# vrgamegirl19/comfyui-vrgamedevgirl

Measured on AMD Instinct MI355X. Metric: Mpixels/s (grain+LUT+colormatch+sharpen) at 4K, higher is better.
Workload: dtype f32

## Files before the change

### comfyui-vrgamedevgirl_amd/csrc/vrg_apply_body.hpp

```cpp
#pragma once
#include "vrg_chain_stages.hpp"
#include "vrg_lanes.hpp"

namespace vrg {

#define VRG_APPLY_ROWS 60
constexpr int APPLY_ROWS = VRG_APPLY_ROWS;
constexpr int APPLY_COLS = 62;
static_assert(APPLY_ROWS % 3 == 0, "APPLY_ROWS must be a multiple of 3");

__device__ __forceinline__ float am_prev(float v) { return tap_prev(v); }
__device__ __forceinline__ float am_next(float v) { return tap_next(v); }

struct AmRow { float l[3], c[3], r[3]; };

#define VRG_APPLY_EARLY_LOAD 1
template <int STAGES, class MATH, bool GENERAL = true>
__device__ __forceinline__ void apply_march_body(uint32_t vblock, uint32_t vgrid, const px3* __restrict__ in, px3* __restrict__ out, int32_t H, int32_t W,
                                                 int32_t strips_x, int32_t segs_y, uint32_t total_waves, const ChainK& D, const MATH& PT) {
    const uint32_t groups = (total_waves + 3u) / 4u;
    const uint32_t per_xcd = (groups + 7u) / 8u;
    const int lane = threadIdx.x & 63;
    const bool zero = D.zero_border != 0;
    const int64_t ppf = (int64_t)H * W;
    const float n0[3] = {0.0f, 0.0f, 0.0f};
    for (uint32_t slot = vblock >> 3; slot < per_xcd; slot += (vgrid >> 3)) {
    const uint32_t grp = (vblock & 7u) * per_xcd + slot;
    if (grp >= groups) break;
    const uint32_t wv = (uint32_t)__builtin_amdgcn_readfirstlane((int)(grp * 4u + (threadIdx.x >> 6)));
    if (wv >= total_waves) break;
    const uint32_t strip = wv % (uint32_t)strips_x;
    const uint32_t rest = wv / (uint32_t)strips_x;
    const uint32_t seg = rest % (uint32_t)segs_y;
    const int64_t f = rest / (uint32_t)segs_y;
    int32_t x0 = (int32_t)strip * APPLY_COLS, y0 = (int32_t)seg * APPLY_ROWS;
    if (W >= APPLY_COLS) x0 = x0 < W - APPLY_COLS ? x0 : W - APPLY_COLS;
    if (H >= APPLY_ROWS) y0 = y0 < H - APPLY_ROWS ? y0 : H - APPLY_ROWS;
    const int32_t rows = H >= APPLY_ROWS ? APPLY_ROWS : H;
    const int32_t x = x0 - 1 + lane;
    const bool x_in = x >= 0 && x < W;
    const int32_t xc = x < 0 ? 0 : (x > W - 1 ? W - 1 : x);
    const bool stores = lane >= 1 && lane <= APPLY_COLS && x_in;
    const px3* fin = in + f * ppf;
    px3* fout = out + f * ppf;
    __amdgpu_buffer_rsrc_t frame_rsrc, in_rsrc;
    if (!GENERAL) {
        const uint64_t fb = reinterpret_cast<uint64_t>(fout);
        const uint64_t fbu = ((uint64_t)(uint32_t)__builtin_amdgcn_readfirstlane((int)(fb >> 32)) << 32) | (uint32_t)__builtin_amdgcn_readfirstlane((int)(uint32_t)fb);
        frame_rsrc = __builtin_amdgcn_make_buffer_rsrc(reinterpret_cast<void*>(fbu), 0, (int)(ppf * 12), 0x00020000);
        const uint64_t ib = reinterpret_cast<uint64_t>(fin);
        const uint64_t ibu = ((uint64_t)(uint32_t)__builtin_amdgcn_readfirstlane((int)(ib >> 32)) << 32) | (uint32_t)__builtin_amdgcn_readfirstlane((int)(uint32_t)ib);
        in_rsrc = __builtin_amdgcn_make_buffer_rsrc(reinterpret_cast<void*>(ibu), 0, (int)(ppf * 12), 0x00020000);
    }
    const FrameCtx FC = frame_ctx<STAGES>(D, f);
    const uint32_t x_bytes = (uint32_t)xc * 12u;
    const uint32_t store_bytes = stores ? (uint32_t)x * 12u : 0x80000000u;

    auto load = [&](int32_t y) {
        const int32_t yc = y < 0 ? 0 : (y > H - 1 ? H - 1 : y);
        if (!GENERAL) {
            typedef unsigned u3 __attribute__((ext_vector_type(3)));
            const u3 v = __builtin_amdgcn_raw_buffer_load_b96(in_rsrc, (int)x_bytes, (int)((uint32_t)(yc * W) * 12u), 0);
            return px3{__uint_as_float(v.x), __uint_as_float(v.y), __uint_as_float(v.z)};
        }
        return fin[(int64_t)yc * W + xc];
    };
    auto process = [&](const px3& v, int32_t y) {
        AmRow r;
        const float xi[3] = {v.r, v.g, v.b};
        float o[3];
        chain_apply_stages<STAGES, !GENERAL>(D, FC, xi, n0, o, PT);
        r.c[0] = o[0]; r.c[1] = o[1]; r.c[2] = o[2];
        if (zero) {
            asm volatile("" ::: "memory");
            const bool inside = x_in && y >= 0 && y < H;
#pragma unroll
            for (int c = 0; c < 3; ++c) r.c[c] = inside ? r.c[c] : 0.0f;
        }
#pragma unroll
        for (int c = 0; c < 3; ++c) {
            r.l[c] = am_prev(r.c[c]);
            r.r[c] = am_next(r.c[c]);
        }
        return r;
    };
    auto emit = [&](int32_t y, const AmRow& a, const AmRow& b, const AmRow& c) {
        float res[3];
        if (STAGES & VRG_STAGE_COLORMATCH) {
            const float p[3][3][3] = {{{a.l[0], a.c[0], a.r[0]}, {b.l[0], b.c[0], b.r[0]}, {c.l[0], c.c[0], c.r[0]}},
                                      {{a.l[1], a.c[1], a.r[1]}, {b.l[1], b.c[1], b.r[1]}, {c.l[1], c.c[1], c.r[1]}},
                                      {{a.l[2], a.c[2], a.r[2]}, {b.l[2], b.c[2], b.r[2]}, {c.l[2], c.c[2], c.r[2]}}};
            stencil_value3_unit<!GENERAL>(D.stencil_op, p, D.strength, D.zero_border, res);
        } else {
#pragma unroll
            for (int ch = 0; ch < 3; ++ch) {
                const float p[3][3] = {{a.l[ch], a.c[ch], a.r[ch]}, {b.l[ch], b.c[ch], b.r[ch]}, {c.l[ch], c.c[ch], c.r[ch]}};
                res[ch] = stencil_value(D.stencil_op, p, D.strength, D.zero_border);
            }
        }
        if (GENERAL) {
            if (stores && y < y0 + rows) fout[(int64_t)y * W + x] = px3{res[0], res[1], res[2]};
        } else {
            typedef unsigned u3 __attribute__((ext_vector_type(3)));
            __builtin_amdgcn_raw_buffer_store_b96(u3{__float_as_uint(res[0]), __float_as_uint(res[1]), __float_as_uint(res[2])}, frame_rsrc, (int)store_bytes,
                                                  (int)((uint32_t)(y * W) * 12u), 0);
        }
    };

    AmRow r0 = process(load(y0 - 1), y0 - 1);
    AmRow r1 = process(load(y0), y0);
    AmRow r2;
    const int32_t y1 = y0 + rows;
    px3 q = load(y0 + 1);
    if (!GENERAL && VRG_APPLY_EARLY_LOAD) {
        for (int32_t y = y0; y < y1; y += 3) {
            const px3 a = load(y + 2);
            r2 = process(q, y + 1);
            emit(y, r0, r1, r2);
            const px3 b = load(y + 3);
            r0 = process(a, y + 2);
            emit(y + 1, r1, r2, r0);
            q = load(y + 4);
            r1 = process(b, y + 3);
            emit(y + 2, r2, r0, r1);
        }
    } else {
        for (int32_t y = y0; y < y1; y += 3) {
            r2 = process(q, y + 1);
            q = load(y + 2);
            emit(y, r0, r1, r2);
            r0 = process(q, y + 2);
            q = load(y + 3);
            emit(y + 1, r1, r2, r0);
            r1 = process(q, y + 3);
            q = load(y + 4);
            emit(y + 2, r2, r0, r1);
        }
    }
    }
}


}
```

### comfyui-vrgamedevgirl_amd/csrc/vrg_torch_stats.hip

```cpp
#include <atomic>
#include "vrg_tstats_body.hpp"
#include "vrg_tstats_config.hpp"

namespace vrg {

template <class OP, class LOAD>
static __device__ __forceinline__ typename OP::acc_t ts_thread_reduce(LOAD X, int64_t n, int shift, bool vectorize, int T, int t, int tx,
                                                                      bool tail_ok) {
    constexpr int VEC = OP::VEC;
    typename OP::acc_t acc[VEC];
#pragma unroll
    for (int i = 0; i < VEC; ++i) acc[i] = OP::ident();
    if (vectorize) {
        int64_t start = 0, end = n;
        if (shift > 0) {
            if (tx >= shift && tx < VEC && tail_ok) acc[0] = OP::template reduce<true>(acc[0], X((int64_t)(tx - shift)));
            start = VEC - shift;
            end = n + shift - VEC;
        }
        for (int64_t idx = t; idx * VEC + VEC - 1 < end; idx += T) {
            const int64_t p = start + idx * VEC;
            acc[0] = OP::template reduce<false>(acc[0], X(p));
#pragma unroll
            for (int i = 1; i < VEC; ++i) acc[i] = OP::template reduce<true>(acc[i], X(p + i));
        }
        const int64_t tail_start = end - end % VEC;
        if (tail_ok && tail_start + tx < end) acc[0] = OP::template reduce<true>(acc[0], X(start + tail_start + tx));
    } else {
        int64_t idx = t;
        while (idx + (int64_t)(VEC - 1) * T < n) {
#pragma unroll
            for (int i = 0; i < VEC; ++i) acc[i] = OP::template reduce<true>(acc[i], X(idx + (int64_t)i * T));
            idx += (int64_t)T * VEC;
        }
#pragma unroll
        for (int i = 0; i < VEC; ++i) {
            if (idx < n) acc[i] = OP::template reduce<true>(acc[i], X(idx));
            idx += T;
        }
    }
#pragma unroll
    for (int i = 1; i < VEC; ++i) acc[0] = OP::combine(acc[0], acc[i]);
    return acc[0];
}

template <class OP, int WHICH>
__global__ void __launch_bounds__(512) k_tstats_plane(const float* __restrict__ lab, int64_t n, int64_t plane0, int chunk_frames, TsCfg cfg,
                                                      float factor, float eps, float* __restrict__ out) {
    __shared__ typename OP::acc_t lds[512];
    const int64_t plane = plane0 + blockIdx.x;
    const int64_t f = plane / 3;
    const int c = (int)(plane % 3);
    const int64_t o_in_call = (f % chunk_frames) * 3 + c;
    const int shift = cfg.vectorize ? (int)((o_in_call * n) % OP::VEC) : 0;
    const int rows = cfg.split ? cfg.bh : 1;
    const int T = cfg.bw * rows;
    const int t = threadIdx.x;
    const bool live = t < T;
    const float* base = lab + (size_t)f * (size_t)n * 3 + c;
    auto X = [base](int64_t p) { return base[(size_t)p * 3]; };
    typename OP::acc_t v = OP::ident();
    if (live) v = ts_thread_reduce<OP>(X, n, shift, cfg.vectorize != 0, T, t, t % cfg.bw, cfg.split ? (t / cfg.bw == 0) : true);
    v = ts_block_reduce<OP>(v, cfg.bw, cfg.bh, cfg.split != 0, t, live, lds);
    if (t == 0) {
        if constexpr (WHICH == 0) out[(size_t)f * 6 + c * 2] = v * factor;
        else out[(size_t)f * 6 + c * 2 + 1] = welf_std(v) + eps;
    }
}

template <int DEPTH>
__global__ void __launch_bounds__(256) k_tstats_rows(const float* __restrict__ lab, int64_t n, int64_t frames, int bw, int bh, TsRows* __restrict__ rows) {
    __shared__ Welf lds_w[256];
    tstats_rows_body<DEPTH>(blockIdx.x, lab, n, frames, bw, bh, rows, lds_w);
}

__global__ void __launch_bounds__(64) k_tstats_rows_finish(const TsRows* __restrict__ rows, int64_t frames, int bh, float factor, float eps,
                                                          float* __restrict__ out) {
    const int64_t i = (int64_t)blockIdx.x * 64 + threadIdx.x;
    if (i >= frames * 6) return;
    const int64_t f = i / 6;
    const int c = (int)(i % 6) >> 1, which = (int)(i & 1);
    if (which == 0) {
        float v[8];
        for (int r = 0; r < bh; ++r) v[r] = rows[f].m[c][r];
        for (int off = bh / 2; off > 0; off >>= 1)
            for (int ty = 0; ty < off; ++ty) v[ty] = MeanOp::combine(v[ty], v[ty + off]);
        out[(size_t)f * 6 + c * 2] = v[0] * factor;
    } else {
        Welf v[8];
        for (int r = 0; r < bh; ++r) v[r] = rows[f].w[c][r];
        for (int off = bh / 2; off > 0; off >>= 1)
            for (int ty = 0; ty < off; ++ty) v[ty] = WelfOp::combine(v[ty], v[ty + off]);
        out[(size_t)f * 6 + c * 2 + 1] = welf_std(v[0]) + eps;
    }
}

struct TsLaneRec { float mean, m2; int cnt; int pad; };
struct TsLanes { TsLaneRec w[3][2][512]; float m[3][512]; };
constexpr int TS_LANES_MAX_STEPS = 16384;

#define VRG_TS_LANES_DEPTH 8
#define VRG_TS_LANES_MEAN_DEPTH 12
#define VRG_TS_LANES_MAX_FRAMES 2

template <bool FUSED, bool FAST, int DEPTH>
static __device__ __forceinline__ bool ts_lane_chain(const float* __restrict__ ub, uint32_t lane_bytes, int steps, bool extra, const float2* __restrict__ tab,
                                                     Welf& acc, int& cnt) {
    bool bad = false;
    acc = WelfOp::ident();
    float xb[DEPTH];
    const int last = steps > 0 ? steps - 1 : 0;
    auto load = [&](int k) {
        const int kk = k < last ? k : last;
        return *reinterpret_cast<const float*>(reinterpret_cast<const char*>(ub + (size_t)kk * 3072) + lane_bytes);
    };
#pragma unroll
    for (int i = 0; i < DEPTH; ++i) xb[i] = load(i);
    int k0 = 0;
    for (; k0 + DEPTH <= steps; k0 += DEPTH) {
#pragma unroll
        for (int i = 0; i < DEPTH; ++i) {
            const float2 t = tab[k0 + i];
            ts_welf_update<FUSED, FAST>(acc, xb[i], t.x, t.y, bad);
            xb[i] = load(k0 + i + DEPTH);
        }
    }
#pragma unroll
    for (int i = 0; i < DEPTH; ++i)
        if (k0 + i < steps) {
            const float2 t = tab[k0 + i];
            ts_welf_update<FUSED, FAST>(acc, xb[i], t.x, t.y, bad);
        }
    cnt = steps;
    if (extra) {
        const float2 t = tab[steps];
        const float x = *reinterpret_cast<const float*>(reinterpret_cast<const char*>(ub + (size_t)steps * 3072) + lane_bytes);
        ts_welf_update<FUSED, FAST>(acc, x, t.x, t.y, bad);
        cnt = steps + 1;
    }
    return bad;
}

template <int DEPTH>
__global__ void __launch_bounds__(448) k_tstats_lanes(const float* __restrict__ lab, int64_t n, int64_t frames, TsLanes* __restrict__ recs) {
    extern __shared__ __attribute__((aligned(16))) float2 ts_rn_tab[];
    const int64_t w = blockIdx.x;
    const int64_t f = (w & 7) + 8 * (w >> 6);
    const int j = (int)((w >> 3) & 7);
    if (f >= frames) return;
    const int wave = __builtin_amdgcn_readfirstlane((int)(threadIdx.x >> 6)), lane = threadIdx.x & 63;
    const int t = 64 * j + lane;
    const int64_t nvw = n / 2, nvm = n / 4;
    const int64_t wsteps = nvw / 512;
    const bool wextra = (int64_t)t < nvw - wsteps * 512;
    for (int64_t i = threadIdx.x; i <= wsteps; i += 448) {
        const float nf = (float)(i + 1);
        ts_rn_tab[i] = float2{nf, 1.0f / nf};
    }
    __syncthreads();
    const float* base = lab + (size_t)f * (size_t)n * 3;
    TsLanes* R = recs + f;
    bool bad = false;
    Welf acc = WelfOp::ident();
    int cnt = 0;
    const bool fast = VRG_TS_MARKSTEIN && wsteps + 2 <= TS_MARKSTEIN_MAX_COUNT;
    const int c = wave >> 1, a = wave & 1;
    const float* ub = base + (wave < 6 ? a * 3 + c : 0);
    const uint32_t lane_bytes = (uint32_t)t * 24u;
    const int ws = (int)wsteps;
    if (wave < 6) {
        if (fast) bad = a ? ts_lane_chain<true, true, DEPTH>(ub, lane_bytes, ws, wextra, ts_rn_tab, acc, cnt) : ts_lane_chain<false, true, DEPTH>(ub, lane_bytes, ws, wextra, ts_rn_tab, acc, cnt);
        else if (a) ts_lane_chain<true, false, DEPTH>(ub, lane_bytes, ws, wextra, ts_rn_tab, acc, cnt);
        else ts_lane_chain<false, false, DEPTH>(ub, lane_bytes, ws, wextra, ts_rn_tab, acc, cnt);
    } else {
        float ma[3][4];
#pragma unroll
        for (int cc = 0; cc < 3; ++cc)
#pragma unroll
            for (int i = 0; i < 4; ++i) ma[cc][i] = 0.0f;
        auto mean_vec = [&](const f32x4& a0, const f32x4& a1, const f32x4& a2) {
            const float e[12] = {a0.x, a0.y, a0.z, a0.w, a1.x, a1.y, a1.z, a1.w, a2.x, a2.y, a2.z, a2.w};
#pragma unroll
            for (int i = 0; i < 4; ++i)
#pragma unroll
                for (int cc = 0; cc < 3; ++cc) ma[cc][i] = ma[cc][i] + e[i * 3 + cc];
        };
        constexpr int MD = VRG_TS_LANES_MEAN_DEPTH;
        const int64_t msteps = nvm / 512;
        const bool mextra = (int64_t)t < nvm - msteps * 512;
        const int64_t last = msteps > 0 ? msteps - 1 : 0;
        f32x4 mb[MD][3];
        auto mload = [&](int i, int64_t r) {
            const f32x4* q = reinterpret_cast<const f32x4*>(base + (size_t)(r * 512 + t) * 12);
            mb[i][0] = q[0]; mb[i][1] = q[1]; mb[i][2] = q[2];
        };
#pragma unroll
        for (int i = 0; i < MD; ++i) mload(i, i < last ? i : last);
        int64_t r0 = 0;
        for (; r0 + MD <= msteps; r0 += MD) {
#pragma unroll
            for (int i = 0; i < MD; ++i) {
                mean_vec(mb[i][0], mb[i][1], mb[i][2]);
                const int64_t nx = r0 + i + MD;
                mload(i, nx < last ? nx : last);
            }
        }
#pragma unroll
        for (int i = 0; i < MD; ++i)
            if (r0 + i < msteps) mean_vec(mb[i][0], mb[i][1], mb[i][2]);
        if (mextra) {
            const f32x4* q = reinterpret_cast<const f32x4*>(base + (size_t)(msteps * 512 + t) * 12);
            mean_vec(q[0], q[1], q[2]);
        }
#pragma unroll
        for (int cc = 0; cc < 3; ++cc) {
            float m = ma[cc][0];
            m = m + ma[cc][1];
            m = m + ma[cc][2];
            m = m + ma[cc][3];
            R->m[cc][t] = m;
        }
    }
    if (fast && __syncthreads_or(bad ? 1 : 0)) {
        if (wave < 6) {
            if (a) ts_lane_chain<true, false, DEPTH>(ub, lane_bytes, ws, wextra, ts_rn_tab, acc, cnt);
            else ts_lane_chain<false, false, DEPTH>(ub, lane_bytes, ws, wextra, ts_rn_tab, acc, cnt);
        }
    }
    if (wave < 6) R->w[c][a][t] = TsLaneRec{acc.mean, acc.m2, cnt, 0};
}

__global__ void __launch_bounds__(512) k_tstats_lanes_finish(const TsLanes* __restrict__ recs, int bw, int bh, float factor, float eps, float* __restrict__ out) {
    __shared__ Welf lds_w[512];
    float* lds_m = reinterpret_cast<float*>(lds_w);
    const int64_t f = blockIdx.x;
    const int t = threadIdx.x;
    const TsLanes* R = recs + f;
    float* o6 = out + (size_t)f * 6;
#pragma unroll
    for (int c = 0; c < 3; ++c) {
        float m = R->m[c][t];
        m = ts_block_reduce<MeanOp>(m, bw, bh, true, t, true, lds_m);
        if (t == 0) o6[c * 2] = m * factor;
    }
#pragma unroll
    for (int c = 0; c < 3; ++c) {
        const TsLaneRec r0 = R->w[c][0][t], r1 = R->w[c][1][t];
        const Welf w0{r0.mean, r0.m2, r0.cnt, (float)r0.cnt}, w1{r1.mean, r1.m2, r1.cnt, (float)r1.cnt};
        Welf w = WelfOp::combine(w0, w1);
        w = ts_block_reduce<WelfOp>(w, bw, bh, true, t, true, lds_w);
        if (t == 0) o6[c * 2 + 1] = welf_std(w) + eps;
    }
}

template <bool SPLIT, int DEPTH>
__global__ void __launch_bounds__(512) k_tstats_frame(const float* __restrict__ lab, int64_t n, int64_t frames, int bw, int bh, float factor,
                                                      float eps, float* __restrict__ out) {
    __shared__ Welf lds_w[512];
    if constexpr (!SPLIT) {
        const int64_t f = blockIdx.x;
        ts_frame_part<-1, DEPTH>(lab + (size_t)f * (size_t)n * 3, n, bw, bh, factor, eps, out + (size_t)f * 6, lds_w);
    } else {
        const int64_t w = blockIdx.x;
        const int64_t f = (w & 7) + 8 * (w >> 5);
        const int part = (int)((w >> 3) & 3);
        if (f >= frames) return;
        const float* base = lab + (size_t)f * (size_t)n * 3;
        float* o6 = out + (size_t)f * 6;
        switch (part) {
            case 0: ts_frame_part<0, DEPTH>(base, n, bw, bh, factor, eps, o6, lds_w); break;
            case 1: ts_frame_part<1, DEPTH>(base, n, bw, bh, factor, eps, o6, lds_w); break;
            case 2: ts_frame_part<2, DEPTH>(base, n, bw, bh, factor, eps, o6, lds_w); break;
            default: ts_frame_part<3, DEPTH>(base, n, bw, bh, factor, eps, o6, lds_w); break;
        }
    }
}

static int ts_launch_planes(const float* lab_call, int64_t n, int64_t o0, int64_t o1, int chunk_frames, float factor, float eps, float* out_call,
                            int num_mp, hipStream_t st) {
    const int64_t O = o1 - o0;
    if (O * n > ((int64_t)1 << 29) && O > 1) {
        const int64_t half = O / 2;
        int rc = ts_launch_planes(lab_call, n, o0, o0 + half, chunk_frames, factor, eps, out_call, num_mp, st);
        if (rc != VRG_OK) return rc;
        return ts_launch_planes(lab_call, n, o0 + half, o1, chunk_frames, factor, eps, out_call, num_mp, st);
    }
    if (O * n > ((int64_t)1 << 29)) return VRG_ERR_UNSUPPORTED;
    TsCfg cm, cw;
    if (!ts_config(O, n, 4, cm, num_mp) || !ts_config(O, n, 2, cw, num_mp)) return VRG_ERR_UNSUPPORTED;
    hipLaunchKernelGGL((k_tstats_plane<MeanOp, 0>), dim3((unsigned)O), dim3(512), 0, st, lab_call, n, o0, chunk_frames, cm, factor, eps, out_call);
    hipLaunchKernelGGL((k_tstats_plane<WelfOp, 1>), dim3((unsigned)O), dim3(512), 0, st, lab_call, n, o0, chunk_frames, cw, factor, eps, out_call);
    VRG_CHECK_LAUNCH();
    return VRG_OK;
}

#define VRG_TS_SPLIT_MAX_FRAMES 64
constexpr int64_t TS_SPLIT_MAX_FRAMES = VRG_TS_SPLIT_MAX_FRAMES;

#define VRG_TS_ROWS_DEPTH 4
#define VRG_TS_SPLIT_DEPTH 2
#define VRG_TS_WHOLE_DEPTH 1
#define VRG_TS_ROWS_MAX_FRAMES 32
constexpr int64_t TS_ROWS_MAX_FRAMES = VRG_TS_ROWS_MAX_FRAMES;

static int ts_launch_calls(const float* lab, int64_t n, int64_t count, int b, float eps, float* out, int num_mp, void* scratch, int64_t scratch_bytes,
                           hipStream_t st, bool prefer_lanes = false) {
    if (count <= 0 || b <= 0) return VRG_OK;
    const int64_t O = (int64_t)b * 3;
    const float factor = (float)O / (float)(O * n);
    if (O * n > ((int64_t)1 << 29)) {
        for (int64_t k = 0; k < count; ++k) {
            const int rc = ts_launch_planes(lab + (size_t)k * b * n * 3, n, 0, O, b, factor, eps, out + (size_t)k * b * 6, num_mp, st);
            if (rc != VRG_OK) return rc;
        }
        return VRG_OK;
    }
    TsCfg cm, cw;
    if (!ts_config(O, n, 4, cm, num_mp) || !ts_config(O, n, 2, cw, num_mp)) return VRG_ERR_UNSUPPORTED;
    const int64_t frames = count * b;
    const bool whole = (n % 4 == 0) && cm.vectorize && cw.vectorize && cm.split && cw.split && cm.bw * cm.bh == 512 && cw.bw * cw.bh == 512 &&
                       cm.bw == cw.bw;
    if (whole) {
#define VRG_TS_LANES 1
        if (VRG_TS_LANES && prefer_lanes && frames <= VRG_TS_LANES_MAX_FRAMES && scratch && scratch_bytes >= frames * (int64_t)sizeof(TsLanes) && cm.bh == cw.bh &&
            n / 1024 + 2 <= TS_LANES_MAX_STEPS && (reinterpret_cast<uintptr_t>(scratch) & 15) == 0) {
            TsLanes* recs = reinterpret_cast<TsLanes*>(scratch);
            const size_t lds = (size_t)(n / 1024 + 2) * sizeof(float2);
            static std::atomic<uint64_t> attr_devices{0};
            int device = 0;
            if (hipGetDevice(&device) != hipSuccess) return VRG_ERR_LAUNCH;
            const uint64_t bit = (device >= 0 && device < 64) ? (1ull << device) : 0;
            if (!(attr_devices.load(std::memory_order_acquire) & bit)) {
                if (hipFuncSetAttribute(reinterpret_cast<const void*>(k_tstats_lanes<VRG_TS_LANES_DEPTH>), hipFuncAttributeMaxDynamicSharedMemorySize,
                                        TS_LANES_MAX_STEPS * (int)sizeof(float2)) != hipSuccess)
                    return VRG_ERR_LAUNCH;
                attr_devices.fetch_or(bit, std::memory_order_release);
            }
            hipLaunchKernelGGL((k_tstats_lanes<VRG_TS_LANES_DEPTH>), dim3((unsigned)(64 * ((frames + 7) / 8))), dim3(448), lds, st, lab, n, frames, recs);
            hipLaunchKernelGGL(k_tstats_lanes_finish, dim3((unsigned)frames), dim3(512), 0, st, recs, cm.bw, cm.bh, factor, eps, out);
            VRG_CHECK_LAUNCH();
            return VRG_OK;
        }
        if (frames <= TS_ROWS_MAX_FRAMES && scratch && scratch_bytes >= frames * (int64_t)sizeof(TsRows) && cm.bh == cw.bh && cm.bh <= 8 && 256 % cm.bw == 0 &&
            (reinterpret_cast<uintptr_t>(scratch) & 15) == 0) {
            TsRows* rows = reinterpret_cast<TsRows*>(scratch);
            hipLaunchKernelGGL((k_tstats_rows<VRG_TS_ROWS_DEPTH>), dim3((unsigned)(64 * ((frames + 7) / 8))), dim3(256), 0, st, lab, n, frames, cm.bw, cm.bh, rows);
            hipLaunchKernelGGL(k_tstats_rows_finish, dim3((unsigned)((frames * 6 + 63) / 64)), dim3(64), 0, st, rows, frames, cm.bh, factor, eps, out);
            VRG_CHECK_LAUNCH();
            return VRG_OK;
        }
        const bool split = frames <= TS_SPLIT_MAX_FRAMES;
        if (split) {
            hipLaunchKernelGGL((k_tstats_frame<true, VRG_TS_SPLIT_DEPTH>), dim3((unsigned)(32 * ((frames + 7) / 8))), dim3(512), 0, st, lab, n, frames, cm.bw,
                               cm.bh, factor, eps, out);
        } else {
            const int64_t per = num_mp > 0 ? num_mp : 256;
            for (int64_t f0 = 0; f0 < frames; f0 += per) {
                const int64_t nf = frames - f0 < per ? frames - f0 : per;
                hipLaunchKernelGGL((k_tstats_frame<false, VRG_TS_WHOLE_DEPTH>), dim3((unsigned)nf), dim3(512), 0, st, lab + (size_t)f0 * (size_t)n * 3, n, nf,
                                   cm.bw, cm.bh, factor, eps, out + (size_t)f0 * 6);
            }
        }
    } else {
        hipLaunchKernelGGL((k_tstats_plane<MeanOp, 0>), dim3((unsigned)(frames * 3)), dim3(512), 0, st, lab, n, (int64_t)0, b, cm, factor, eps, out);
        hipLaunchKernelGGL((k_tstats_plane<WelfOp, 1>), dim3((unsigned)(frames * 3)), dim3(512), 0, st, lab, n, (int64_t)0, b, cw, factor, eps, out);
    }
    VRG_CHECK_LAUNCH();
    return VRG_OK;
}

}

extern "C" int64_t vrg_lab_stats_torch_scratch_bytes(int64_t frames) {
    if (frames <= 0 || frames > vrg::TS_ROWS_MAX_FRAMES) return 0;
    return frames * (int64_t)(sizeof(vrg::TsLanes) > sizeof(vrg::TsRows) ? sizeof(vrg::TsLanes) : sizeof(vrg::TsRows));
}

extern "C" int vrg_lab_stats_torch_f32(const float* lab, int64_t frames, int32_t height, int32_t width, int32_t chunk_frames,
                                       float* mean_std, float eps, void* stream) {
    return vrg_lab_stats_torch_ws_f32(lab, frames, height, width, chunk_frames, mean_std, eps, nullptr, 0, stream);
}

static int lab_stats_torch_any(const float* lab, int64_t frames, int32_t height, int32_t width, int32_t chunk_frames, float* mean_std, float eps, void* scratch,
                               int64_t scratch_bytes, void* stream, bool prefer_lanes);

extern "C" int vrg_lab_stats_torch_ws_f32(const float* lab, int64_t frames, int32_t height, int32_t width, int32_t chunk_frames,
                                          float* mean_std, float eps, void* scratch, int64_t scratch_bytes, void* stream) {
    return lab_stats_torch_any(lab, frames, height, width, chunk_frames, mean_std, eps, scratch, scratch_bytes, stream, false);
}

extern "C" int vrg_lab_stats_torch_lat_f32(const float* lab, int64_t frames, int32_t height, int32_t width, int32_t chunk_frames,
                                           float* mean_std, float eps, void* scratch, int64_t scratch_bytes, void* stream) {
    return lab_stats_torch_any(lab, frames, height, width, chunk_frames, mean_std, eps, scratch, scratch_bytes, stream, true);
}

static int lab_stats_torch_any(const float* lab, int64_t frames, int32_t height, int32_t width, int32_t chunk_frames, float* mean_std, float eps, void* scratch,
                               int64_t scratch_bytes, void* stream, bool prefer_lanes) {
    using namespace vrg;
    if (frames < 0 || height <= 0 || width <= 0 || chunk_frames <= 0) return VRG_ERR_BAD_ARG;
    if (frames == 0) return VRG_OK;
    if (!lab || !mean_std) return VRG_ERR_BAD_ARG;
    int dev = 0, cus = 0;
    if (hipGetDevice(&dev) != hipSuccess) return VRG_ERR_NO_DEVICE;
    if (hipDeviceGetAttribute(&cus, hipDeviceAttributeMultiprocessorCount, dev) != hipSuccess) return VRG_ERR_NO_DEVICE;
    if (cus <= 0) return VRG_ERR_NO_DEVICE;
    if (cus < 100) return VRG_ERR_UNSUPPORTED;
    const int64_t n = (int64_t)height * width;
    if (frames * 3 > 0x7fffffff / 2) return VRG_ERR_UNSUPPORTED;
    hipStream_t st = (hipStream_t)stream;
    const int64_t full = frames / chunk_frames;
    const int tail = (int)(frames % chunk_frames);
    int rc = ts_launch_calls(lab, n, full, chunk_frames, eps, mean_std, cus, scratch, scratch_bytes, st, prefer_lanes);
    if (rc != VRG_OK) return rc;
    if (tail) rc = ts_launch_calls(lab + (size_t)full * chunk_frames * n * 3, n, 1, tail, eps, mean_std + (size_t)full * chunk_frames * 6, cus, scratch, scratch_bytes, st, prefer_lanes);
    return rc;
}
```

### comfyui-vrgamedevgirl_amd/csrc/vrg_tstats_body.hpp

```cpp
#pragma once
#include "vrg_common.hpp"

namespace vrg {

struct Welf { float mean, m2; int n; float nf; };

struct MeanOp {
    typedef float acc_t;
    static constexpr int VEC = 4;
    static __device__ __forceinline__ acc_t ident() { return 0.0f; }
    template <bool FUSED> static __device__ __forceinline__ acc_t reduce(acc_t a, float x) { return a + x; }
    static __device__ __forceinline__ acc_t combine(acc_t a, acc_t b) { return a + b; }
    static __device__ __forceinline__ acc_t shfl_down(acc_t a, int off) { return __shfl_down(a, off, 64); }
};

struct WelfOp {
    typedef Welf acc_t;
    static constexpr int VEC = 2;
    static __device__ __forceinline__ acc_t ident() { return Welf{0.0f, 0.0f, 0, 0.0f}; }
    template <bool FUSED> static __device__ __forceinline__ acc_t reduce(acc_t a, float x) {
        const int n1 = a.n + 1;
        const float nf1 = (float)n1;
        const float delta = x - a.mean;
        const float mean1 = a.mean + delta / nf1;
        const float d2 = x - mean1;
        const float m2 = FUSED ? __builtin_fmaf(delta, d2, a.m2) : a.m2 + delta * d2;
        return Welf{mean1, m2, n1, nf1};
    }
    static __device__ __forceinline__ acc_t combine(acc_t a, acc_t b) {
        if (a.nf == 0.0f) return b;
        if (b.nf == 0.0f) return a;
        const float delta = b.mean - a.mean;
        const float cnt = a.nf + b.nf;
        const float nb = b.nf / cnt;
        const float mean = __builtin_fmaf(delta, nb, a.mean);
        const float m2 = __builtin_fmaf((delta * delta) * a.nf, nb, a.m2 + b.m2);
        return Welf{mean, m2, -1, cnt};
    }
    static __device__ __forceinline__ acc_t shfl_down(acc_t a, int off) {
        return Welf{__shfl_down(a.mean, off, 64), __shfl_down(a.m2, off, 64), __shfl_down(a.n, off, 64), __shfl_down(a.nf, off, 64)};
    }
};

static __device__ __forceinline__ float welf_std(const Welf& a) {
    const float divisor = a.nf > 1.0f ? a.nf - 1.0f : 0.0f;
    return __builtin_sqrtf(a.m2 / divisor);
}

template <class OP>
static __device__ typename OP::acc_t ts_block_reduce(typename OP::acc_t v, int bw, int bh, bool split, int t, bool live,
                                                     typename OP::acc_t* lds) {
    const int tx = t % bw, ty = t / bw;
    int dim_x = bw;
    __syncthreads();
    if (dim_x > 64) {
        if (live) lds[t] = v;
        for (int off = dim_x / 2; off >= 64; off >>= 1) {
            __syncthreads();
            if (live && tx < off && tx + off < bw) {
                v = OP::combine(v, lds[t + off]);
                lds[t] = v;
            }
        }
        dim_x = 64;
    }
    __syncthreads();
    for (int off = 1; off < dim_x; off <<= 1) {
        const typename OP::acc_t other = OP::shfl_down(v, off);
        v = OP::combine(v, other);
    }
    if (split) {
        if (live) lds[t] = v;
        for (int off = bh / 2; off > 0; off >>= 1) {
            __syncthreads();
            if (live && ty < off && ty + off < bh) {
                v = OP::combine(v, lds[t + off * bw]);
                lds[t] = v;
            }
        }
    }
    return v;
}


template <int PART>
struct TsRound {
    static constexpr bool MEAN = PART == -1 || PART == 3;
    static constexpr bool WELF = PART != 3;
    static constexpr int NC = PART == -1 ? 3 : 1;
    f32x4 m[MEAN ? 3 : 1];
    float w[WELF ? 2 * 2 * NC : 1];
    __device__ __forceinline__ void load(const float* __restrict__ base, int64_t r, int t) {
        if constexpr (MEAN) {
            const f32x4* q = reinterpret_cast<const f32x4*>(base + (size_t)(r * 512 + t) * 12);
            m[0] = q[0]; m[1] = q[1]; m[2] = q[2];
        }
        if constexpr (WELF) {
#pragma unroll
            for (int s = 0; s < 2; ++s) {
                const float* q = base + (size_t)(r * 1024 + s * 512 + t) * 6;
                if constexpr (PART == -1) {
                    const float2* q2 = reinterpret_cast<const float2*>(q);
                    const float2 b0 = q2[0], b1 = q2[1], b2 = q2[2];
                    w[s * 6 + 0] = b0.x; w[s * 6 + 1] = b0.y; w[s * 6 + 2] = b1.x; w[s * 6 + 3] = b1.y; w[s * 6 + 4] = b2.x; w[s * 6 + 5] = b2.y;
                } else {
                    w[s * 2 + 0] = q[PART];
                    w[s * 2 + 1] = q[3 + PART];
                }
            }
        }
    }
};

struct TsRows { Welf w[3][8]; float m[3][8]; };

struct TsAcc {
    float ma[3][4];
    Welf wa[3][2];
    int cnt;
};

static __device__ __forceinline__ bool ts_delta_safe(float d) {
    const float a = __builtin_fabsf(d);
    return ((a >= 0x1p-100f) & (a <= 0x1p+100f)) | (d == 0.0f);
}

template <bool FUSED, bool FAST>
static __device__ __forceinline__ void ts_welf_update(Welf& a, float x, float nf1, float rn, bool& bad) {
    const float delta = x - a.mean;
    float q;
    if (FAST) {
        bad = bad | !ts_delta_safe(delta);
        const float q0 = delta * rn;
        const float e = __builtin_fmaf(-nf1, q0, delta);
        q = __builtin_fmaf(e, rn, q0);
    } else {
        q = delta / nf1;
    }
    const float mean1 = a.mean + q;
    const float d2 = x - mean1;
    a.m2 = FUSED ? __builtin_fmaf(delta, d2, a.m2) : a.m2 + delta * d2;
    a.mean = mean1;
}

template <int PART, int TS_DEPTH, bool FAST>
static __device__ __forceinline__ bool ts_accumulate(const float* __restrict__ base, int64_t n, int t, TsAcc& A) {
    typedef TsRound<PART> R;
    constexpr int NC = R::NC, C0 = PART == -1 ? 0 : (PART == 3 ? 0 : PART);
    const int64_t nvm = n / 4, nvw = n / 2;
    bool bad = false;
#pragma unroll
    for (int c = 0; c < 3; ++c) {
#pragma unroll
        for (int i = 0; i < 4; ++i) A.ma[c][i] = 0.0f;
        A.wa[c][0] = WelfOp::ident(); A.wa[c][1] = WelfOp::ident();
    }
    A.cnt = 0;

    auto mean_vec = [&](const f32x4& a0, const f32x4& a1, const f32x4& a2) {
        const float e[12] = {a0.x, a0.y, a0.z, a0.w, a1.x, a1.y, a1.z, a1.w, a2.x, a2.y, a2.z, a2.w};
#pragma unroll
        for (int i = 0; i < 4; ++i)
#pragma unroll
            for (int c = 0; c < 3; ++c) A.ma[c][i] = A.ma[c][i] + e[i * 3 + c];
    };
    auto welf_vec = [&](const float* e) {
        const int n1 = A.cnt + 1;
        const float nf1 = (float)n1;
        const float rn = FAST ? 1.0f / nf1 : 0.0f;
#pragma unroll
        for (int c = 0; c < NC; ++c) {
            ts_welf_update<false, FAST>(A.wa[c][0], e[c], nf1, rn, bad);
            ts_welf_update<true, FAST>(A.wa[c][1], e[NC + c], nf1, rn, bad);
        }
        A.cnt = n1;
    };
    const int64_t rounds = nvm / 512;
    R buf[TS_DEPTH];
    auto process = [&](const R& b) {
        if constexpr (R::MEAN) mean_vec(b.m[0], b.m[1], b.m[2]);
        if constexpr (R::WELF) { welf_vec(b.w); welf_vec(b.w + 2 * NC); }
    };
    if constexpr (TS_DEPTH == 1) {
        if (rounds > 0) buf[0].load(base, 0, t);
        for (int64_t r = 0; r < rounds; ++r) {
            process(buf[0]);
            if (r + 1 < rounds) buf[0].load(base, r + 1, t);
        }
    } else if (rounds > 0) {
        const int64_t last = rounds - 1;
#pragma unroll
        for (int i = 0; i < TS_DEPTH; ++i) buf[i].load(base, i < last ? i : last, t);
        int64_t r0 = 0;
        for (; r0 + TS_DEPTH <= rounds; r0 += TS_DEPTH) {
#pragma unroll
            for (int i = 0; i < TS_DEPTH; ++i) {
                process(buf[i]);
                const int64_t nx = r0 + i + TS_DEPTH;
                buf[i].load(base, nx < last ? nx : last, t);
            }
        }
#pragma unroll
        for (int i = 0; i < TS_DEPTH; ++i)
            if (r0 + i < rounds) process(buf[i]);
    }
    if constexpr (R::MEAN)
        for (int64_t idx = rounds * 512 + t; idx < nvm; idx += 512) {
            const f32x4* q = reinterpret_cast<const f32x4*>(base + (size_t)idx * 12);
            mean_vec(q[0], q[1], q[2]);
        }
    if constexpr (R::WELF)
        for (int64_t idx = rounds * 1024 + t; idx < nvw; idx += 512) {
            const float* q = base + (size_t)idx * 6;
            float e[2 * NC];
#pragma unroll
            for (int c = 0; c < NC; ++c) { e[c] = q[C0 + c]; e[NC + c] = q[3 + C0 + c]; }
            welf_vec(e);
        }
#pragma unroll
    for (int c = 0; c < NC; ++c) {
        A.wa[c][0].n = A.cnt; A.wa[c][0].nf = (float)A.cnt;
        A.wa[c][1].n = A.cnt; A.wa[c][1].nf = (float)A.cnt;
    }
    return bad;
}

#define VRG_TS_MARKSTEIN 1
constexpr int64_t TS_MARKSTEIN_MAX_COUNT = 1 << 20;

template <int PART, int TS_DEPTH, bool ROWS = false>
static __device__ void ts_frame_part(const float* __restrict__ base, int64_t n, int bw, int bh, float factor, float eps, float* __restrict__ o6,
                                     Welf* lds_w, int t0 = 0, TsRows* rows_out = nullptr) {
    typedef TsRound<PART> R;
    constexpr int NC = R::NC, C0 = PART == -1 ? 0 : (PART == 3 ? 0 : PART);
    float* lds_m = reinterpret_cast<float*>(lds_w);
    const int t = t0 + (int)threadIdx.x;
    TsAcc A;
    if (VRG_TS_MARKSTEIN && R::WELF && n / 1024 + 2 <= TS_MARKSTEIN_MAX_COUNT) {
        const bool bad = ts_accumulate<PART, TS_DEPTH, true>(base, n, t, A);
        if (__syncthreads_or(bad ? 1 : 0)) ts_accumulate<PART, TS_DEPTH, false>(base, n, t, A);
    } else {
        ts_accumulate<PART, TS_DEPTH, false>(base, n, t, A);
    }
    float (&ma)[3][4] = A.ma;
    Welf (&wa)[3][2] = A.wa;
    const int tl = (int)threadIdx.x;
    if constexpr (R::MEAN) {
#pragma unroll
        for (int c = 0; c < 3; ++c) {
            float m = ma[c][0];
            m = m + ma[c][1];
            m = m + ma[c][2];
            m = m + ma[c][3];
            if constexpr (ROWS) {
                m = ts_block_reduce<MeanOp>(m, bw, bh, false, tl, true, lds_m);
                if (tl % bw == 0) rows_out->m[c][t / bw] = m;
            } else {
                m = ts_block_reduce<MeanOp>(m, bw, bh, true, t, true, lds_m);
                if (t == 0) o6[c * 2] = m * factor;
            }
        }
    }
    if constexpr (R::WELF) {
#pragma unroll
        for (int c = 0; c < NC; ++c) {
            Welf w = WelfOp::combine(wa[c][0], wa[c][1]);
            if constexpr (ROWS) {
                w = ts_block_reduce<WelfOp>(w, bw, bh, false, tl, true, lds_w);
                if (tl % bw == 0) rows_out->w[C0 + c][t / bw] = w;
            } else {
                w = ts_block_reduce<WelfOp>(w, bw, bh, true, t, true, lds_w);
                if (t == 0) o6[(C0 + c) * 2 + 1] = welf_std(w) + eps;
            }
        }
    }
}

template <int DEPTH>
__device__ __forceinline__ void tstats_rows_body(int64_t w, const float* __restrict__ lab, int64_t n, int64_t frames, int bw, int bh,
                                                 TsRows* __restrict__ rows, Welf* lds_w) {
    const int64_t f = (w & 7) + 8 * (w >> 6);
    const int sub = (int)((w >> 3) & 7), part = sub >> 1, t0 = (sub & 1) * 256;
    if (f >= frames) return;
    const float* base = lab + (size_t)f * (size_t)n * 3;
    TsRows* ro = rows + f;
    switch (part) {
        case 0: ts_frame_part<0, DEPTH, true>(base, n, bw, bh, 0.0f, 0.0f, nullptr, lds_w, t0, ro); break;
        case 1: ts_frame_part<1, DEPTH, true>(base, n, bw, bh, 0.0f, 0.0f, nullptr, lds_w, t0, ro); break;
        case 2: ts_frame_part<2, DEPTH, true>(base, n, bw, bh, 0.0f, 0.0f, nullptr, lds_w, t0, ro); break;
        default: ts_frame_part<3, DEPTH, true>(base, n, bw, bh, 0.0f, 0.0f, nullptr, lds_w, t0, ro); break;
    }
}

}
```

Before: 43700.

## Stage whole-frame stats rounds through an LDS ring and enlarge apply row tiles

Adds a shared-memory double-buffered path to the whole-frame statistics reduction. Each thread stores its 48-byte vector load into an LDS ring, accumulates the mean from registers, then reads the data back in the pixel-pair layout the Welford update needs, so the global buffer is read once per round. It also triples the rows each apply wave marches, which amortises the halo rows and setup per wave but leaves fewer waves in flight. The ring costs extra LDS and a barrier per round.

```diff
diff --git a/comfyui-vrgamedevgirl_amd/csrc/vrg_apply_body.hpp b/comfyui-vrgamedevgirl_amd/csrc/vrg_apply_body.hpp
--- a/comfyui-vrgamedevgirl_amd/csrc/vrg_apply_body.hpp
+++ b/comfyui-vrgamedevgirl_amd/csrc/vrg_apply_body.hpp
@@ -4,7 +4,7 @@
 
 namespace vrg {
 
-#define VRG_APPLY_ROWS 60
+#define VRG_APPLY_ROWS 180
 constexpr int APPLY_ROWS = VRG_APPLY_ROWS;
 constexpr int APPLY_COLS = 62;
 static_assert(APPLY_ROWS % 3 == 0, "APPLY_ROWS must be a multiple of 3");
diff --git a/comfyui-vrgamedevgirl_amd/csrc/vrg_torch_stats.hip b/comfyui-vrgamedevgirl_amd/csrc/vrg_torch_stats.hip
--- a/comfyui-vrgamedevgirl_amd/csrc/vrg_torch_stats.hip
+++ b/comfyui-vrgamedevgirl_amd/csrc/vrg_torch_stats.hip
@@ -258,8 +258,9 @@
                                                       float eps, float* __restrict__ out) {
     __shared__ Welf lds_w[512];
     if constexpr (!SPLIT) {
+        __shared__ __attribute__((aligned(16))) float ring[2 * TS_ROUND_FLOATS];
         const int64_t f = blockIdx.x;
-        ts_frame_part<-1, DEPTH>(lab + (size_t)f * (size_t)n * 3, n, bw, bh, factor, eps, out + (size_t)f * 6, lds_w);
+        ts_frame_part<-1, DEPTH, false, true>(lab + (size_t)f * (size_t)n * 3, n, bw, bh, factor, eps, out + (size_t)f * 6, lds_w, 0, nullptr, ring);
     } else {
         const int64_t w = blockIdx.x;
         const int64_t f = (w & 7) + 8 * (w >> 5);
diff --git a/comfyui-vrgamedevgirl_amd/csrc/vrg_tstats_body.hpp b/comfyui-vrgamedevgirl_amd/csrc/vrg_tstats_body.hpp
--- a/comfyui-vrgamedevgirl_amd/csrc/vrg_tstats_body.hpp
+++ b/comfyui-vrgamedevgirl_amd/csrc/vrg_tstats_body.hpp
@@ -143,8 +143,11 @@
     a.mean = mean1;
 }
 
-template <int PART, int TS_DEPTH, bool FAST>
-static __device__ __forceinline__ bool ts_accumulate(const float* __restrict__ base, int64_t n, int t, TsAcc& A) {
+constexpr int TS_ROUND_FLOATS = 2048 * 3;
+
+template <int PART, int TS_DEPTH, bool FAST, bool SHARED = false>
+static __device__ __forceinline__ bool ts_accumulate(const float* __restrict__ base, int64_t n, int t, TsAcc& A, float* ring = nullptr) {
+    static_assert(!SHARED || PART == -1, "the shared fetch is the whole-frame form's");
     typedef TsRound<PART> R;
     constexpr int NC = R::NC, C0 = PART == -1 ? 0 : (PART == 3 ? 0 : PART);
     const int64_t nvm = n / 4, nvw = n / 2;
@@ -181,7 +184,42 @@
         if constexpr (R::MEAN) mean_vec(b.m[0], b.m[1], b.m[2]);
         if constexpr (R::WELF) { welf_vec(b.w); welf_vec(b.w + 2 * NC); }
     };
-    if constexpr (TS_DEPTH == 1) {
+    if constexpr (SHARED) {
+        if (rounds > 0) {
+            const int64_t last = rounds - 1;
+            f32x4 pre[TS_DEPTH][3];
+            auto fetch = [&](f32x4 (&p)[3], int64_t r) {
+                const f32x4* q = reinterpret_cast<const f32x4*>(base + (size_t)(r * 512 + t) * 12);
+                p[0] = q[0]; p[1] = q[1]; p[2] = q[2];
+            };
+            auto step = [&](f32x4 (&p)[3], int64_t r, int64_t nx) {
+                float* slot = ring + (r & 1) * TS_ROUND_FLOATS;
+                f32x4* sw = reinterpret_cast<f32x4*>(slot + t * 12);
+                sw[0] = p[0]; sw[1] = p[1]; sw[2] = p[2];
+                mean_vec(p[0], p[1], p[2]);
+                fetch(p, nx < last ? nx : last);
+                __syncthreads();
+                float w[12];
+#pragma unroll
+                for (int s = 0; s < 2; ++s) {
+                    const float2* q2 = reinterpret_cast<const float2*>(slot + (s * 512 + t) * 6);
+                    const float2 b0 = q2[0], b1 = q2[1], b2 = q2[2];
+                    w[s * 6 + 0] = b0.x; w[s * 6 + 1] = b0.y; w[s * 6 + 2] = b1.x; w[s * 6 + 3] = b1.y; w[s * 6 + 4] = b2.x; w[s * 6 + 5] = b2.y;
+                }
+                welf_vec(w); welf_vec(w + 6);
+            };
+#pragma unroll
+            for (int i = 0; i < TS_DEPTH; ++i) fetch(pre[i], i < last ? i : last);
+            int64_t r0 = 0;
+            for (; r0 + TS_DEPTH <= rounds; r0 += TS_DEPTH) {
+#pragma unroll
+                for (int i = 0; i < TS_DEPTH; ++i) step(pre[i], r0 + i, r0 + i + TS_DEPTH);
+            }
+#pragma unroll
+            for (int i = 0; i < TS_DEPTH; ++i)
+                if (r0 + i < rounds) step(pre[i], r0 + i, last);
+        }
+    } else if constexpr (TS_DEPTH == 1) {
         if (rounds > 0) buf[0].load(base, 0, t);
         for (int64_t r = 0; r < rounds; ++r) {
             process(buf[0]);
@@ -228,19 +266,19 @@
 #define VRG_TS_MARKSTEIN 1
 constexpr int64_t TS_MARKSTEIN_MAX_COUNT = 1 << 20;
 
-template <int PART, int TS_DEPTH, bool ROWS = false>
+template <int PART, int TS_DEPTH, bool ROWS = false, bool SHARED = false>
 static __device__ void ts_frame_part(const float* __restrict__ base, int64_t n, int bw, int bh, float factor, float eps, float* __restrict__ o6,
-                                     Welf* lds_w, int t0 = 0, TsRows* rows_out = nullptr) {
+                                     Welf* lds_w, int t0 = 0, TsRows* rows_out = nullptr, float* ring = nullptr) {
     typedef TsRound<PART> R;
     constexpr int NC = R::NC, C0 = PART == -1 ? 0 : (PART == 3 ? 0 : PART);
     float* lds_m = reinterpret_cast<float*>(lds_w);
     const int t = t0 + (int)threadIdx.x;
     TsAcc A;
     if (VRG_TS_MARKSTEIN && R::WELF && n / 1024 + 2 <= TS_MARKSTEIN_MAX_COUNT) {
-        const bool bad = ts_accumulate<PART, TS_DEPTH, true>(base, n, t, A);
-        if (__syncthreads_or(bad ? 1 : 0)) ts_accumulate<PART, TS_DEPTH, false>(base, n, t, A);
+        const bool bad = ts_accumulate<PART, TS_DEPTH, true, SHARED>(base, n, t, A, ring);
+        if (__syncthreads_or(bad ? 1 : 0)) ts_accumulate<PART, TS_DEPTH, false, SHARED>(base, n, t, A, ring);
     } else {
-        ts_accumulate<PART, TS_DEPTH, false>(base, n, t, A);
+        ts_accumulate<PART, TS_DEPTH, false, SHARED>(base, n, t, A, ring);
     }
     float (&ma)[3][4] = A.ma;
     Welf (&wa)[3][2] = A.wa;
```

Result: no change. 44160 (median of 6 runs) (+1.1%).
